# akashsengupta1997/HierarchicalProbabilistic3DHuman

Hardware: AMD Instinct MI355X
Metric: images/sec end-to-end (num_samples=100) (higher is better)
Workload: dtype f32

## Files before the change

### hierarchicalprobabilistic3dhuman_amd/csrc/api.hip

```cpp
#include <stdarg.h>

#include "hps_common.h"

namespace hps {
static thread_local char g_err[512] = "";

void set_error(const char* fmt, ...) {
    va_list ap;
    va_start(ap, fmt);
    vsnprintf(g_err, sizeof(g_err), fmt, ap);
    va_end(ap);
}
}

extern "C" int hps_version(void) { return 502; }

extern "C" int64_t hps_query_workspace(int what, int64_t d0, int64_t d1, int64_t d2) {
    if (d0 < 0 || d1 < 0 || d2 < 0) { hps::set_error("hps_query_workspace: negative dimension"); return -1; }
    const int64_t f = (int64_t)sizeof(float);
    auto up = [](int64_t x, int64_t m) { return (x + m - 1) / m * m; };
    switch (what) {
        case HPS_WS_CONV_SPLITK: return d0 <= 1 ? 0 : d0 * d1 * d2 * f;
        case HPS_WS_SMPL_MP: return up(d0, 128);
        case HPS_WS_SMPL_XT: return d1 * up(d0, 128) * f;
        case HPS_WS_SMPL_A: return d0 * d1 * 12 * f;
        case HPS_WS_SMPL_VPOSED: return d0 * up(3 * d1, 128) * f;
        case HPS_WS_HEAD_F: return d0 * d1 * 9 * f;
        case HPS_WS_HEAD_USV: return d0 * d1 * 21 * f;
        case HPS_WS_MF_LOSS: return hps::mf_loss_ws_bytes(d0);
        case HPS_WS_SMPL_LBS_BWD: return hps::lbs_backward_ws_bytes(d0, d1, d2);
        case HPS_WS_SMPL_BLEND_BWD: return hps::blend_backward_ws_bytes(d0, d1, d2);
        case HPS_WS_HEAD_LEVELS_BWD: return hps::head_levels_backward_ws_bytes(d0, d1, d2);
        case HPS_WS_HEAD_TRUNK_BWD: return hps::head_trunk_backward_ws_bytes(d0, d1, d2);
        case HPS_WS_SEG_BBOX: return d0 * 32 * 4 * (int64_t)sizeof(int32_t);
#ifdef HPS_DEV_BUILD
        case HPS_DEV_WS_HEAD_SYNC: return ((d0 + 3) / 4) * (HPS_HEAD_MAX_LEVELS + 1) * (int64_t)sizeof(int32_t);
#endif
        case HPS_WS_RENDER: return hps::render_ws_bytes(d0, d1, d2);
        case HPS_WS_SILHOUETTE: {
            const int64_t faces = d2 & 0xffffffffll, W = d2 >> 32;
            if (faces > (1 << 24) || W < 1 || W > 4096) { hps::set_error("hps_query_workspace: HPS_WS_SILHOUETTE takes d2 = faces + W * 2^32 with faces <= 2^24, W in [1, 4096]"); return -1; }
            return hps::silhouette_ws_bytes(d0, d1, faces, W);
        }
        case HPS_WS_TRAIN_METRICS: return hps::train_metrics_ws_bytes(d0);
        default: hps::set_error("hps_query_workspace: unknown item %d", what); return -1;
    }
}
extern "C" const char* hps_last_error(void) { return hps::g_err; }

extern "C" int hps_stream_create_cu_partition(int first_cu, int num_cus, hps_stream_t* stream_out) {
    if (!stream_out) return hps::bad_arg("hps_stream_create_cu_partition: null pointer");
    int dev = 0;
    hipError_t e = hipGetDevice(&dev);
    hipDeviceProp_t prop;
    if (e == hipSuccess) e = hipGetDeviceProperties(&prop, dev);
    if (e != hipSuccess) { hps::set_error("hps_stream_create_cu_partition: %s", hipGetErrorString(e)); return (int)e; }
    const int total = prop.multiProcessorCount, n_xcd = 8;
    const int per_xcd = total / n_xcd;
    if (total % n_xcd != 0 || first_cu < 0 || num_cus < 1 || first_cu + num_cus > per_xcd)
        return hps::bad_arg("hps_stream_create_cu_partition: CU range outside [0, CUs per XCD)");
    uint32_t mask[16] = {0};
    for (int c = first_cu; c < first_cu + num_cus; ++c)
        for (int x = 0; x < n_xcd; ++x) {
            const int bit = c * n_xcd + x;
            mask[bit / 32] |= 1u << (bit % 32);
        }
    hipStream_t s = nullptr;
    e = hipExtStreamCreateWithCUMask(&s, (uint32_t)((total + 31) / 32), mask);
    if (e != hipSuccess) { hps::set_error("hipExtStreamCreateWithCUMask: %s", hipGetErrorString(e)); return (int)e; }
    *stream_out = (hps_stream_t)s;
    return HPS_OK;
}

extern "C" int hps_stream_destroy(hps_stream_t stream) {
    const hipError_t e = hipStreamDestroy((hipStream_t)stream);
    if (e != hipSuccess) { hps::set_error("hipStreamDestroy: %s", hipGetErrorString(e)); return (int)e; }
    return HPS_OK;
}
```

### hierarchicalprobabilistic3dhuman_amd/csrc/conv_pad.hip

```cpp
#include <type_traits>

#include "hps_common.h"

namespace hps {

typedef float f32x16 __attribute__((ext_vector_type(16)));

constexpr int PBK = 32;

__device__ __forceinline__ unsigned fastdiv(unsigned n, unsigned d, unsigned magic) {
    unsigned q = __umulhi(n, magic);
    if (n - q * d >= d) ++q;
    return q;
}
static unsigned div_magic(unsigned d) { return d <= 1 ? 0xffffffffu : (unsigned)(0x100000000ull / d); }

__device__ __forceinline__ void lds_dma16_sv(unsigned voff, const float* sbase, unsigned lds_addr) {
    unsigned keep;
    asm volatile("s_mov_b32 %0, m0\n\ts_mov_b32 m0, %3\n\ts_nop 0\n\tglobal_load_lds_dwordx4 %1, %2\n\ts_mov_b32 m0, %0"
                 : "=&s"(keep)
                 : "v"(voff), "s"(sbase), "s"(lds_addr)
                 : "memory");
}

struct PadGeom {
    int img_pitch, row_pitch, pix_pitch;
    int cin_k;
    int kw;
    int stride, off;
    int Ho, Wo, Mtot, Kp, Cout;
    int opad;
    int relu, tiles_m, ksplit;
    unsigned magic_howo, magic_wo;
    int ablate;
};
struct DownArgs {
    const float* wn;
    const float* scale;
    const float* shift;
    float* y;
    int blocks_main;
    int tap_kh, tap_kw;
};
struct NoDown {};

#ifdef HPS_DEV_BUILD
static int g_pad_ablate = 0;
#else
constexpr int g_pad_ablate = 0;
#endif

__device__ __forceinline__ unsigned out_pixel_offset(unsigned m, const PadGeom& g) {
    const unsigned howo = (unsigned)(g.Ho * g.Wo);
    const unsigned b = fastdiv(m, howo, g.magic_howo), rem = m - b * howo;
    const unsigned ho = fastdiv(rem, (unsigned)g.Wo, g.magic_wo), wo = rem - ho * g.Wo;
    return ((b * (g.Ho + 2 * g.opad) + ho + g.opad) * (g.Wo + 2 * g.opad) + wo + g.opad) * (unsigned)g.Cout;
}

template <int BM, int BN, int WM, int WN, int ST = 2, bool DOWN = false>
__global__ __launch_bounds__(256) void conv_pad_kernel(const float* __restrict__ x, const float* __restrict__ wn,
                                                       const float* __restrict__ scale, const float* __restrict__ shift,
                                                       const float* __restrict__ residual, float* __restrict__ y,
                                                       float* __restrict__ partial, const PadGeom g,
                                                       const std::conditional_t<DOWN, DownArgs, NoDown> d) {
    constexpr int WAVES_N = BN / WN;
    constexpr int TM = WM / 32, TN = WN / 32;
    constexpr int A_LD = BM / 32, B_LD = BN / 32;
    static_assert((BM / WM) * (BN / WN) == 4, "4 waves per workgroup");
    typedef __attribute__((address_space(3))) void* lptr_t;

    extern __shared__ __attribute__((aligned(16))) float smem[];
    float* sA = smem;
    float* sB = smem + ST * BM * PBK;

    int bx = blockIdx.x;
    bool down = false;
    if constexpr (DOWN) {
        if (bx >= d.blocks_main) {
            if (blockIdx.y != 0) return;
            down = true;
            bx -= d.blocks_main;
            wn = d.wn; scale = d.scale; shift = d.shift; y = d.y; residual = nullptr;
        }
    }
    const int filter_kp = down ? g.cin_k : g.Kp;
    const int ksplit = down ? 1 : g.ksplit;
    const int relu = down ? 0 : g.relu;
    const int tile_n = bx / g.tiles_m, tile_m = bx % g.tiles_m;
    const int m0 = tile_m * BM, n0 = tile_n * BN;
    const int tid = threadIdx.x, lane = tid & 63, wave = tid >> 6;
    const int wm0 = (wave / WAVES_N) * WM, wn0 = (wave % WAVES_N) * WN;
    const int kl = lane >> 5, il = lane & 31;
    const int drow = wave * 8 + (lane >> 3);
    const int dquad = ((lane & 7) ^ ((drow >> 1) & 7)) * 4;

    unsigned a_off[A_LD], b_off[B_LD];
    {
        const unsigned howo = (unsigned)(g.Ho * g.Wo);
#pragma unroll
        for (int r = 0; r < A_LD; ++r) {
            const unsigned m = (unsigned)(m0 + drow + 32 * r);
            unsigned o = 0;
            if (m < (unsigned)g.Mtot) {
                const unsigned b = fastdiv(m, howo, g.magic_howo), rem = m - b * howo;
                const unsigned ho = fastdiv(rem, (unsigned)g.Wo, g.magic_wo), wo = rem - ho * g.Wo;
                o = b * g.img_pitch + (ho * g.stride + g.off) * g.row_pitch + (wo * g.stride + g.off) * g.pix_pitch;
            }
            a_off[r] = (o + dquad) * 4u;
        }
#pragma unroll
        for (int r = 0; r < B_LD; ++r) b_off[r] = ((unsigned)(n0 + drow + 32 * r) * filter_kp + dquad) * 4u;
    }

    f32x16 acc[TM][TN];
#pragma unroll
    for (int i = 0; i < TM; ++i)
#pragma unroll
        for (int j = 0; j < TN; ++j)
#pragma unroll
            for (int r = 0; r < 16; ++r) acc[i][j][r] = 0.0f;

    const int chunks_total = filter_kp / PBK;
    const int per_split = chunks_total / ksplit;
    const int c_begin = down ? 0 : blockIdx.y * per_split, c_end = c_begin + per_split;
    const int cpt = g.cin_k / PBK;
    int ci = c_begin % cpt, tap = c_begin / cpt;
    int kw = tap % g.kw, kh = tap / g.kw;
    if constexpr (DOWN) {
        if (down) { kh = d.tap_kh; kw = d.tap_kw; }
    }
    const float* a_src = x + (size_t)kh * g.row_pitch + (size_t)kw * g.pix_pitch + (size_t)ci * PBK;
    const float* b_src = wn + (size_t)c_begin * PBK;
    const int tap_jump = g.pix_pitch - g.cin_k + PBK;
    const int row_jump = g.row_pitch - (g.kw - 1) * g.pix_pitch - g.cin_k + PBK;

    const unsigned lds_a = (unsigned)(size_t)(lptr_t)(sA + wave * 8 * PBK);
    const unsigned lds_b = (unsigned)(size_t)(lptr_t)(sB + wave * 8 * PBK);
    auto advance = [&]() {
        b_src += PBK;
        if (++ci < cpt) a_src += PBK;
        else {
            ci = 0;
            if (++kw < g.kw) a_src += tap_jump;
            else { kw = 0; a_src += row_jump; }
        }
    };
    auto dma_chunk = [&](int buf) {
        const unsigned la = __builtin_amdgcn_readfirstlane(lds_a + buf * BM * PBK * 4);
        const unsigned lb = __builtin_amdgcn_readfirstlane(lds_b + buf * BN * PBK * 4);
#pragma unroll
        for (int r = 0; r < A_LD; ++r) lds_dma16_sv(a_off[r], a_src, la + r * 32 * PBK * 4);
#pragma unroll
        for (int r = 0; r < B_LD; ++r) lds_dma16_sv(b_off[r], b_src, lb + r * 32 * PBK * 4);
        advance();
    };
    auto dma_piece = [&](int p, const float* pa_src, const float* pb_src, unsigned la, unsigned lb) {
        if (p < A_LD) lds_dma16_sv(a_off[p < A_LD ? p : 0], pa_src, la + p * 32 * PBK * 4);
        else if (p < A_LD + B_LD) lds_dma16_sv(b_off[p >= A_LD && p < A_LD + B_LD ? p - A_LD : 0], pb_src, lb + (p - A_LD) * 32 * PBK * 4);
    };

    const int fsw = (il >> 1) & 7;
#ifdef HPS_DEV_BUILD
    if (g.ablate >= 2) {
        if (((blockIdx.x >> 8) & 1) && blockIdx.x < 512)
            for (int i = 0; i < (g.ablate - 1) * 1; ++i) __builtin_amdgcn_s_sleep(127);
    }
#endif
    dma_chunk(0);
#pragma unroll
    for (int q = 1; q < ST - 1; ++q)
        if (c_begin + q < c_end) dma_chunk(q);
    for (int c = c_begin; c < c_end; ++c) {
        const int buf = ST == 2 ? (c - c_begin) & 1 : (c - c_begin) % ST;
        {
            const int younger = min(ST - 2, c_end - 1 - c);
            if (ST >= 4 && younger >= 2) asm volatile("s_waitcnt vmcnt(%0)" ::"n"(2 * (A_LD + B_LD)) : "memory");
            else if (ST >= 3 && younger >= 1) asm volatile("s_waitcnt vmcnt(%0)" ::"n"(A_LD + B_LD) : "memory");
            else asm volatile("s_waitcnt vmcnt(0)" ::: "memory");
        }
        __syncthreads();
        static_assert(A_LD + B_LD <= (PBK / 8) * TM * TN, "one DMA piece per accumulator block of a chunk at most");
#ifdef HPS_DEV_BUILD
        const bool spread = g.ablate != 3 || ST != 2;
#else
        constexpr bool spread = true;
#endif
        const bool more = c + (ST - 1) < c_end;
        const float* na_src = a_src;
        const float* nb_src = b_src;
        const int nbuf = ST == 2 ? buf ^ 1 : (c - c_begin + ST - 1) % ST;
        const unsigned nla = __builtin_amdgcn_readfirstlane(lds_a + nbuf * BM * PBK * 4);
        const unsigned nlb = __builtin_amdgcn_readfirstlane(lds_b + nbuf * BN * PBK * 4);
        if (more) {
            if (spread) advance();
            else dma_chunk(buf ^ 1);
        }
        const float* pa = sA + (size_t)buf * BM * PBK + (wm0 + il) * PBK;
        const float* pb = sB + (size_t)buf * BN * PBK + (wn0 + il) * PBK;
        float4 a4[2][TM], b4[2][TN];
        auto load_frags = [&](int gq, int s) {
            const int slot = ((2 * gq + kl) ^ fsw) * 4;
#pragma unroll
            for (int i = 0; i < TM; ++i) a4[s][i] = *reinterpret_cast<const float4*>(pa + i * 32 * PBK + slot);
#pragma unroll
            for (int j = 0; j < TN; ++j) b4[s][j] = *reinterpret_cast<const float4*>(pb + j * 32 * PBK + slot);
        };
        load_frags(0, 0);
#pragma unroll
        for (int gq = 0; gq < PBK / 8; ++gq) {
            if (gq + 1 < PBK / 8) load_frags(gq + 1, (gq + 1) & 1);
            __builtin_amdgcn_sched_barrier(0);
#pragma unroll
            for (int i = 0; i < TM; ++i)
#pragma unroll
                for (int j = 0; j < TN; ++j) {
                    acc[i][j] = __builtin_amdgcn_mfma_f32_32x32x2f32(b4[gq & 1][j].x, a4[gq & 1][i].x, acc[i][j], 0, 0, 0);
                    acc[i][j] = __builtin_amdgcn_mfma_f32_32x32x2f32(b4[gq & 1][j].y, a4[gq & 1][i].y, acc[i][j], 0, 0, 0);
                    acc[i][j] = __builtin_amdgcn_mfma_f32_32x32x2f32(b4[gq & 1][j].z, a4[gq & 1][i].z, acc[i][j], 0, 0, 0);
                    acc[i][j] = __builtin_amdgcn_mfma_f32_32x32x2f32(b4[gq & 1][j].w, a4[gq & 1][i].w, acc[i][j], 0, 0, 0);
                    if (spread && more) {
                        __builtin_amdgcn_sched_barrier(0);
                        dma_piece((gq * TM + i) * TN + j, na_src, nb_src, nla, nlb);
                        __builtin_amdgcn_sched_barrier(0);
                    }
                }
            __builtin_amdgcn_sched_barrier(0);
        }
    }

    if (ksplit > 1) {
        float* dst = partial + (size_t)blockIdx.y * g.Mtot * g.Cout;
#pragma unroll
        for (int i = 0; i < TM; ++i) {
            const int m = m0 + wm0 + i * 32 + il;
            if (m >= g.Mtot) continue;
#pragma unroll
            for (int j = 0; j < TN; ++j)
#pragma unroll
                for (int q = 0; q < 4; ++q)
                    *reinterpret_cast<float4*>(dst + (size_t)m * g.Cout + n0 + wn0 + j * 32 + 8 * q + 4 * kl) =
                        make_float4(acc[i][j][4 * q], acc[i][j][4 * q + 1], acc[i][j][4 * q + 2], acc[i][j][4 * q + 3]);
        }
        return;
    }

    if (g.ablate == 1) {
        float t = 0.0f;
#pragma unroll
        for (int i = 0; i < TM; ++i)
#pragma unroll
            for (int j = 0; j < TN; ++j)
#pragma unroll
                for (int r = 0; r < 16; ++r) t += acc[i][j][r];
        if (t == 12345.678f) y[0] = t;
        return;
    }

    constexpr int EP = WN + 4;
    constexpr int LPP = WN / 4;
    constexpr int PPI = 64 / LPP;
    static_assert(4 * 32 * EP <= ST * (BM + BN) * PBK, "the epilogue patches fit in the K-loop buffers");
    __syncthreads();
    float* patch = smem + wave * 32 * EP;
    const int c4 = (lane % LPP) * 4;
    const int co = n0 + wn0 + c4;
    const float4 sc = *reinterpret_cast<const float4*>(scale + co), sh = *reinterpret_cast<const float4*>(shift + co);
#pragma unroll
    for (int i = 0; i < TM; ++i) {
#pragma unroll
        for (int j = 0; j < TN; ++j)
#pragma unroll
            for (int q = 0; q < 4; ++q)
                *reinterpret_cast<float4*>(patch + il * EP + j * 32 + 8 * q + 4 * kl) =
                    make_float4(acc[i][j][4 * q], acc[i][j][4 * q + 1], acc[i][j][4 * q + 2], acc[i][j][4 * q + 3]);
        constexpr int U = 32 / PPI;
        if (m0 + BM <= g.Mtot) {
            unsigned po[U];
            float4 a[U];
#pragma unroll
            for (int u = 0; u < U; ++u) {
                po[u] = out_pixel_offset((unsigned)(m0 + wm0 + i * 32 + u * PPI + lane / LPP), g) + (unsigned)co;
                a[u] = *reinterpret_cast<const float4*>(patch + (u * PPI + lane / LPP) * EP + c4);
            }
            if (residual) {
                float4 res[U];
#pragma unroll
                for (int u = 0; u < U; ++u) res[u] = *reinterpret_cast<const float4*>(residual + po[u]);
#pragma unroll
                for (int u = 0; u < U; ++u) {
                    float4 v = make_float4(a[u].x * sc.x + sh.x + res[u].x, a[u].y * sc.y + sh.y + res[u].y,
                                           a[u].z * sc.z + sh.z + res[u].z, a[u].w * sc.w + sh.w + res[u].w);
                    if (relu) { v.x = fmaxf(v.x, 0.f); v.y = fmaxf(v.y, 0.f); v.z = fmaxf(v.z, 0.f); v.w = fmaxf(v.w, 0.f); }
                    *reinterpret_cast<float4*>(y + po[u]) = v;
                }
            } else {
#pragma unroll
                for (int u = 0; u < U; ++u) {
                    float4 v = make_float4(a[u].x * sc.x + sh.x + 0.f, a[u].y * sc.y + sh.y + 0.f, a[u].z * sc.z + sh.z + 0.f,
                                           a[u].w * sc.w + sh.w + 0.f);
                    if (relu) { v.x = fmaxf(v.x, 0.f); v.y = fmaxf(v.y, 0.f); v.z = fmaxf(v.z, 0.f); v.w = fmaxf(v.w, 0.f); }
                    *reinterpret_cast<float4*>(y + po[u]) = v;
                }
            }
            continue;
        }
        unsigned po[U];
        bool live[U];
        float4 res[U];
#pragma unroll
        for (int u = 0; u < U; ++u) {
            const int m = m0 + wm0 + i * 32 + u * PPI + lane / LPP;
            live[u] = m < g.Mtot;
            po[u] = live[u] ? out_pixel_offset((unsigned)m, g) + (unsigned)co : 0u;
            res[u] = (residual && live[u]) ? *reinterpret_cast<const float4*>(residual + po[u]) : make_float4(0.f, 0.f, 0.f, 0.f);
        }
#pragma unroll
        for (int u = 0; u < U; ++u) {
            const float4 a = *reinterpret_cast<const float4*>(patch + (u * PPI + lane / LPP) * EP + c4);
            float4 v = make_float4(a.x * sc.x + sh.x + res[u].x, a.y * sc.y + sh.y + res[u].y, a.z * sc.z + sh.z + res[u].z,
                                   a.w * sc.w + sh.w + res[u].w);
            if (relu) { v.x = fmaxf(v.x, 0.f); v.y = fmaxf(v.y, 0.f); v.z = fmaxf(v.z, 0.f); v.w = fmaxf(v.w, 0.f); }
            if (live[u]) *reinterpret_cast<float4*>(y + po[u]) = v;
        }
    }
}

__global__ __launch_bounds__(256) void splitk_pad_epilogue_kernel(const float* __restrict__ partial,
                                                                  const float* __restrict__ scale,
                                                                  const float* __restrict__ shift,
                                                                  const float* __restrict__ residual,
                                                                  float* __restrict__ y, long total4, const PadGeom g) {
    const long i = (long)blockIdx.x * 256 + threadIdx.x;
    if (i >= total4) return;
    const float4* p4 = reinterpret_cast<const float4*>(partial) + i;
    float4 acc = p4[0];
    int k = 1;
    for (; k + 6 <= g.ksplit; k += 6) {
        float4 v[6];
#pragma unroll
        for (int q = 0; q < 6; ++q) v[q] = p4[(size_t)(k + q) * total4];
#pragma unroll
        for (int q = 0; q < 6; ++q) { acc.x += v[q].x; acc.y += v[q].y; acc.z += v[q].z; acc.w += v[q].w; }
    }
    for (; k < g.ksplit; ++k) {
        const float4 v = p4[(size_t)k * total4];
        acc.x += v.x; acc.y += v.y; acc.z += v.z; acc.w += v.w;
    }
    const unsigned e = (unsigned)(i * 4);
    const unsigned m = e / (unsigned)g.Cout, co = e - m * g.Cout;
    const size_t o = (size_t)out_pixel_offset(m, g) + co;
    const float4 sc = *reinterpret_cast<const float4*>(scale + co), sh = *reinterpret_cast<const float4*>(shift + co);
    float4 v = make_float4(acc.x * sc.x + sh.x, acc.y * sc.y + sh.y, acc.z * sc.z + sh.z, acc.w * sc.w + sh.w);
    if (residual) {
        const float4 r = *reinterpret_cast<const float4*>(residual + o);
        v.x += r.x; v.y += r.y; v.z += r.z; v.w += r.w;
    }
    if (g.relu) { v.x = fmaxf(v.x, 0.f); v.y = fmaxf(v.y, 0.f); v.z = fmaxf(v.z, 0.f); v.w = fmaxf(v.w, 0.f); }
    *reinterpret_cast<float4*>(y + o) = v;
}

template <int C>
__global__ __launch_bounds__(256) void nchw_to_padded_nhwc_kernel(const float* __restrict__ x, float* __restrict__ y,
                                                                  int H, int W, int P, int runs_per_row) {
    __shared__ float sp[256 * C];
    const int t = threadIdx.x;
    const int run = blockIdx.x % runs_per_row;
    const long row = blockIdx.x / runs_per_row;
    const long b = row / H;
    const int h = (int)(row - b * H);
    const int w0 = run * 256, n = min(256, W - w0);
    const long hw = (long)H * W;
    if (t < n) {
        const float* src = x + (b * C) * hw + (long)h * W + w0 + t;
#pragma unroll
        for (int c = 0; c < C; ++c) sp[t * C + c] = src[c * hw];
    }
    __syncthreads();
    float2* dst = reinterpret_cast<float2*>(y + ((b * (H + 2 * P) + h + P) * (long)(W + 2 * P) + w0 + P) * C);
    const float2* s2 = reinterpret_cast<const float2*>(sp);
    for (int i = t; i < n * C / 2; i += 256) dst[i] = s2[i];
}

__global__ __launch_bounds__(256) void nchw_to_padded_nhwc_generic_kernel(const float* __restrict__ x, float* __restrict__ y, int C,
                                                                          int CP, int H, int W, int WF, int P, long total) {
    const long i = (long)blockIdx.x * 256 + threadIdx.x;
    if (i >= total) return;
    const int w = (int)(i % W);
    long r = i / W;
    const int h = (int)(r % H); r /= H;
    const int c = (int)(r % C);
    const long b = r / C;
    y[((b * (H + 2 * P) + h + P) * (long)(WF + 2 * P) + w + P) * CP + c] = x[i];
}

__global__ __launch_bounds__(256) void maxpool_pad_kernel(const float* __restrict__ x, float* __restrict__ y, int H, int W,
                                                          int C, int Ho, int Wo, int opad, long total) {
    const long i = (long)blockIdx.x * 256 + threadIdx.x;
    if (i >= total) return;
    const int c4 = C / 4, Ho2 = (Ho + 1) / 2, Wo2 = (Wo + 1) / 2;
    const int cq = (int)(i % c4);
    long p = i / c4;
    const int wo = 2 * (int)(p % Wo2); p /= Wo2;
    const int ho = 2 * (int)(p % Ho2);
    const long b = p / Ho2;
    float4 v[5][5];
#pragma unroll
    for (int r = 0; r < 5; ++r) {
        const int hi = min(max(ho * 2 - 1 + r, 0), H - 1);
#pragma unroll
        for (int q = 0; q < 5; ++q) {
            const int wi = min(max(wo * 2 - 1 + q, 0), W - 1);
            v[r][q] = *reinterpret_cast<const float4*>(x + ((b * H + hi) * W + wi) * C + cq * 4);
        }
    }
    auto max4 = [](const float4& a, const float4& c) { return make_float4(fmaxf(a.x, c.x), fmaxf(a.y, c.y), fmaxf(a.z, c.z), fmaxf(a.w, c.w)); };
    float4 hm[5][2];
#pragma unroll
    for (int r = 0; r < 5; ++r) {
        hm[r][0] = max4(max4(v[r][0], v[r][1]), v[r][2]);
        hm[r][1] = max4(max4(v[r][2], v[r][3]), v[r][4]);
    }
#pragma unroll
    for (int a = 0; a < 2; ++a)
#pragma unroll
        for (int c = 0; c < 2; ++c) {
            if (ho + a >= Ho || wo + c >= Wo) continue;
            const float4 m = max4(max4(hm[2 * a][c], hm[2 * a + 1][c]), hm[2 * a + 2][c]);
            *reinterpret_cast<float4*>(y + ((b * (Ho + 2 * opad) + ho + a + opad) * (long)(Wo + 2 * opad) + wo + c + opad) * C + cq * 4) = m;
        }
}

__global__ __launch_bounds__(256) void avgpool_pad_kernel(const float* __restrict__ x, float* __restrict__ y, int H, int W,
                                                          int C, int P, int total) {
    const int i = blockIdx.x * 256 + threadIdx.x;
    if (i >= total) return;
    const int b = i / C, c = i % C;
    const int Wp = W + 2 * P;
    const float* s = x + ((size_t)b * (H + 2 * P) + P) * Wp * C + (size_t)P * C + c;
    float acc = 0.0f;
    for (int h = 0; h < H; ++h)
        for (int w0 = 0; w0 < W; w0 += 8) {
            float t[8];
#pragma unroll
            for (int q = 0; q < 8; ++q) t[q] = s[((size_t)h * Wp + min(w0 + q, W - 1)) * C];
#pragma unroll
            for (int q = 0; q < 8; ++q) acc += (w0 + q < W) ? t[q] : 0.0f;
        }
    y[i] = acc / (float)(H * W);
}

template <int BM, int BN, int WM, int WN, int ST = 2>
static int launch_conv_pad(const float* x, const float* wn, const float* scale, const float* shift, const float* residual,
                           float* y, float* partial, PadGeom g, hipStream_t s, const DownArgs* down = nullptr) {
    g.tiles_m = ceil_div(g.Mtot, BM);
    const int tiles_n = g.Cout / BN;
    const size_t lds = (size_t)ST * (BM + BN) * PBK * sizeof(float);
    if (down) {
        DownArgs d = *down;
        d.blocks_main = g.tiles_m * tiles_n;
        if (lds > 64 * 1024)
            if (int rc = grant_lds<&conv_pad_kernel<BM, BN, WM, WN, ST, true>>((int)lds, "hps_conv2d_bn_act_pad_down")) return rc;
        hipLaunchKernelGGL((conv_pad_kernel<BM, BN, WM, WN, ST, true>), dim3(2 * d.blocks_main, g.ksplit), dim3(256), lds, s, x, wn, scale,
                           shift, residual, y, partial, g, d);
    } else {
        if (lds > 64 * 1024)
            if (int rc = grant_lds<&conv_pad_kernel<BM, BN, WM, WN, ST>>((int)lds, "hps_conv2d_bn_act_pad")) return rc;
        hipLaunchKernelGGL((conv_pad_kernel<BM, BN, WM, WN, ST>), dim3(g.tiles_m * tiles_n, g.ksplit), dim3(256), lds, s, x, wn, scale,
                           shift, residual, y, partial, g, NoDown());
    }
    if (g.ksplit > 1) {
        const long total4 = (long)g.Mtot * g.Cout / 4;
        hipLaunchKernelGGL(splitk_pad_epilogue_kernel, dim3((unsigned)((total4 + 255) / 256)), dim3(256), 0, s, partial, scale,
                           shift, residual, y, total4, g);
    }
    return check_launch("hps_conv2d_bn_act_pad");
}

}

using namespace hps;

static int conv_pad_entry(const float* x, const float* wn, const float* scale, const float* shift,
                          const float* residual, float* y, int B, int H, int W, int ipad, int Cin, int Cout,
                          int KH, int KW, int stride, int pad, int opad, int relu, int row_mode, int variant,
                          int ksplit, float* splitk_ws, hps_stream_t stream, DownArgs* down) {
    if (!x || !wn || !scale || !shift || !y) return bad_arg("hps_conv2d_bn_act_pad: null pointer");
    if (ipad < pad || opad < 0) return bad_arg("hps_conv2d_bn_act_pad: the input halo must cover the convolution padding");
    if (Cout % 64 != 0) return bad_arg("hps_conv2d_bn_act_pad: Cout % 64 == 0 required");
    if (B <= 0) return HPS_OK;
    PadGeom g;
    const int Hp = H + 2 * ipad, Wp = W + 2 * ipad;
    g.pix_pitch = Cin;
    g.row_pitch = Wp * Cin;
    g.img_pitch = Hp * g.row_pitch;
    g.stride = stride;
    g.off = ipad - pad;
    g.Ho = (H + 2 * pad - KH) / stride + 1;
    g.Wo = (W + 2 * pad - KW) / stride + 1;
    g.Mtot = B * g.Ho * g.Wo;
    g.Cout = Cout;
    g.opad = opad;
    g.relu = relu;
    g.ksplit = ksplit < 1 ? 1 : ksplit;
    if (row_mode) {
        g.cin_k = ceil_div(KW * Cin, PBK) * PBK;
        g.kw = 1;
        if ((stride * Cin) % 4 != 0 || g.row_pitch % 4 != 0 || (g.off * Cin) % 4 != 0)
            return bad_arg("hps_conv2d_bn_act_pad: row mode needs 16-byte aligned window starts");
        if (((g.Wo - 1) * stride + g.off) * Cin + g.cin_k > g.row_pitch)
            return bad_arg("hps_conv2d_bn_act_pad: row mode window overruns the padded row");
    } else {
        if (Cin % PBK != 0) return bad_arg("hps_conv2d_bn_act_pad: Cin % 32 == 0 required (or row mode)");
        g.cin_k = Cin;
        g.kw = KW;
    }
    g.Kp = KH * g.kw * g.cin_k;
    if ((size_t)B * g.img_pitch * 4 >= 0xffffffffull || (size_t)Cout * g.Kp * 4 >= 0xffffffffull)
        return bad_arg("hps_conv2d_bn_act_pad: tensor exceeds the 32-bit lane offsets");
    if ((g.Kp / PBK) % g.ksplit != 0 || (g.ksplit > 1 && !splitk_ws)) return bad_arg("hps_conv2d_bn_act_pad: ksplit");
    g.magic_howo = div_magic((unsigned)(g.Ho * g.Wo));
    g.magic_wo = div_magic((unsigned)g.Wo);
    g.ablate = g_pad_ablate;
    hipStream_t s = (hipStream_t)stream;
    if (g.ksplit > 1 && variant != 3 && variant != 5) variant = Cout % 128 == 0 ? 1 : 2;
    if (variant == 0) {
        if (Cout % 128 == 0 && ((long)g.Mtot / 128) * (Cout / 128) >= 256) variant = 1;
        else if (Cout == 64 && g.Mtot / 256 >= 512) variant = 4;
        else variant = 3;
    }
    if (variant == 1 && Cout % 128 != 0) variant = 2;
    if (down) {
        switch (variant) {
            case 1: return launch_conv_pad<128, 128, 64, 64>(x, wn, scale, shift, residual, y, splitk_ws, g, s, down);
            case 2: return launch_conv_pad<128, 64, 64, 32>(x, wn, scale, shift, residual, y, splitk_ws, g, s, down);
            case 3: return launch_conv_pad<64, 64, 32, 32>(x, wn, scale, shift, residual, y, splitk_ws, g, s, down);
            case 5: return launch_conv_pad<64, 64, 32, 32, 4>(x, wn, scale, shift, residual, y, splitk_ws, g, s, down);
            default: set_error("hps_conv2d_bn_act_pad_down: tile variant %d carries no down-sample (issue the two convolutions separately)", variant);
                     return HPS_E_UNSUPPORTED;
        }
    }
    switch (variant) {
        case 1: return launch_conv_pad<128, 128, 64, 64>(x, wn, scale, shift, residual, y, splitk_ws, g, s);
        case 2: return launch_conv_pad<128, 64, 64, 32>(x, wn, scale, shift, residual, y, splitk_ws, g, s);
        case 3: return launch_conv_pad<64, 64, 32, 32>(x, wn, scale, shift, residual, y, splitk_ws, g, s);
        case 4: return launch_conv_pad<256, 64, 64, 64>(x, wn, scale, shift, residual, y, splitk_ws, g, s);
        case 5: return launch_conv_pad<64, 64, 32, 32, 4>(x, wn, scale, shift, residual, y, splitk_ws, g, s);
#ifdef HPS_DEV_BUILD
        case 6: return launch_conv_pad<64, 64, 32, 32, 3>(x, wn, scale, shift, residual, y, splitk_ws, g, s);
#endif
        default: return bad_arg("hps_conv2d_bn_act_pad: variant");
    }
}

extern "C" int hps_conv2d_bn_act_pad(const float* x, const float* wn, const float* scale, const float* shift,
                                     const float* residual, float* y, int B, int H, int W, int ipad, int Cin, int Cout,
                                     int KH, int KW, int stride, int pad, int opad, int relu, int row_mode, int variant,
                                     int ksplit, float* splitk_ws, hps_stream_t stream) {
    return conv_pad_entry(x, wn, scale, shift, residual, y, B, H, W, ipad, Cin, Cout, KH, KW, stride, pad, opad, relu, row_mode, variant,
                          ksplit, splitk_ws, stream, nullptr);
}

extern "C" int hps_conv2d_bn_act_pad_down(const float* x, const float* wn, const float* scale, const float* shift, float* y,
                                          const float* wn_down, const float* scale_down, const float* shift_down, float* y_down,
                                          int B, int H, int W, int ipad, int Cin, int Cout, int KH, int KW, int stride, int pad,
                                          int opad, int relu, int variant, int ksplit, float* splitk_ws, hps_stream_t stream) {
    if (!wn_down || !scale_down || !shift_down || !y_down) return bad_arg("hps_conv2d_bn_act_pad_down: null pointer");
    if (KH != KW || KH % 2 != 1 || pad != KH / 2 || stride < 1)
        return bad_arg("hps_conv2d_bn_act_pad_down: the main convolution must be k x k / s / (k / 2) (its centre tap is the 1x1 / s / 0 window)");
    DownArgs d;
    d.wn = wn_down; d.scale = scale_down; d.shift = shift_down; d.y = y_down;
    d.blocks_main = 0;
    d.tap_kh = pad; d.tap_kw = pad;
    return conv_pad_entry(x, wn, scale, shift, nullptr, y, B, H, W, ipad, Cin, Cout, KH, KW, stride, pad, opad, relu, 0, variant, ksplit,
                          splitk_ws, stream, &d);
}

#ifdef HPS_DEV_BUILD
extern "C" int hps_dev_conv_pad_ablate(int mode) {
    g_pad_ablate = mode;
    return HPS_OK;
}
#endif

extern "C" int hps_nchw_to_padded_nhwc(const float* x, float* y, int B, int C, int H, int W, int P, hps_stream_t stream) {
    if (!x || !y) return bad_arg("hps_nchw_to_padded_nhwc: null pointer");
    if (B <= 0 || H <= 0 || W <= 0) return HPS_OK;
    const int runs = ceil_div(W, 256);
    const long blocks = (long)B * H * runs;
    if (blocks > 0x7fffffffL) return bad_arg("hps_nchw_to_padded_nhwc: too many rows");
    hipStream_t s = (hipStream_t)stream;
    if (C == 18) hipLaunchKernelGGL(nchw_to_padded_nhwc_kernel<18>, dim3((unsigned)blocks), dim3(256), 0, s, x, y, H, W, P, runs);
    else if (C == 4) hipLaunchKernelGGL(nchw_to_padded_nhwc_kernel<4>, dim3((unsigned)blocks), dim3(256), 0, s, x, y, H, W, P, runs);
    else if (C == 64) hipLaunchKernelGGL(nchw_to_padded_nhwc_kernel<64>, dim3((unsigned)blocks), dim3(256), 0, s, x, y, H, W, P, runs);
    else return bad_arg("hps_nchw_to_padded_nhwc: C must be 4, 18 or 64");
    return check_launch("hps_nchw_to_padded_nhwc");
}

extern "C" int hps_nchw_to_padded_nhwc_generic(const float* x, float* y, int B, int C, int CP, int H, int W, int WF, int P,
                                               hps_stream_t stream) {
    if (!x || !y) return bad_arg("hps_nchw_to_padded_nhwc_generic: null pointer");
    if (C <= 0 || CP < C || WF < W || P < 0) return bad_arg("hps_nchw_to_padded_nhwc_generic: need CP >= C > 0, WF >= W, P >= 0");
    if (B <= 0 || H <= 0 || W <= 0) return HPS_OK;
    const long total = (long)B * C * H * W;
    if ((total + 255) / 256 > 0x7fffffffL) return bad_arg("hps_nchw_to_padded_nhwc_generic: tensor too large");
    hipLaunchKernelGGL(nchw_to_padded_nhwc_generic_kernel, dim3((unsigned)((total + 255) / 256)), dim3(256), 0, (hipStream_t)stream, x, y,
                       C, CP, H, W, WF, P, total);
    return check_launch("hps_nchw_to_padded_nhwc_generic");
}

extern "C" int hps_maxpool3x3s2_pad(const float* x, float* y, int B, int H, int W, int C, int opad, hps_stream_t stream) {
    if (!x || !y) return bad_arg("hps_maxpool3x3s2_pad: null pointer");
    if (C % 4 != 0) return bad_arg("hps_maxpool3x3s2_pad: C % 4 == 0 required");
    const int Ho = (H + 2 - 3) / 2 + 1, Wo = (W + 2 - 3) / 2 + 1;
    const long total = (long)B * ((Ho + 1) / 2) * ((Wo + 1) / 2) * (C / 4);
    if (total <= 0) return HPS_OK;
    hipLaunchKernelGGL(maxpool_pad_kernel, dim3((unsigned)((total + 255) / 256)), dim3(256), 0, (hipStream_t)stream, x, y, H, W,
                       C, Ho, Wo, opad, total);
    return check_launch("hps_maxpool3x3s2_pad");
}

extern "C" int hps_global_avgpool_pad(const float* x, float* y, int B, int H, int W, int C, int P, hps_stream_t stream) {
    if (!x || !y) return bad_arg("hps_global_avgpool_pad: null pointer");
    const int total = B * C;
    if (total <= 0) return HPS_OK;
    hipLaunchKernelGGL(avgpool_pad_kernel, dim3((total + 255) / 256), dim3(256), 0, (hipStream_t)stream, x, y, H, W, C, P,
                       total);
    return check_launch("hps_global_avgpool_pad");
}
```

### hierarchicalprobabilistic3dhuman_amd/csrc/hps_common.h

```cpp
#pragma once
#include <hip/hip_runtime.h>
#include <stdint.h>
#include <stdio.h>

#include <atomic>

#include "hps.h"
#ifdef HPS_DEV_BUILD
#include "hps_dev.h"
#endif

namespace hps {

void set_error(const char* fmt, ...);

int64_t mf_loss_ws_bytes(int64_t rows);
int64_t lbs_backward_ws_bytes(int64_t M, int64_t V, int64_t J);
int64_t blend_backward_ws_bytes(int64_t M, int64_t kp, int64_t np);
int64_t head_levels_backward_ws_bytes(int64_t B, int64_t total_in, int64_t NJ);
int64_t head_trunk_backward_ws_bytes(int64_t B, int64_t wide, int64_t nt);
int64_t render_ws_bytes(int64_t B, int64_t Nd, int64_t F);
int64_t silhouette_ws_bytes(int64_t M, int64_t Nd, int64_t F, int64_t W);
int64_t train_metrics_ws_bytes(int64_t B);

inline int check_launch(const char* what) {
    hipError_t e = hipGetLastError();
    if (e != hipSuccess) {
        set_error("%s: %s", what, hipGetErrorString(e));
        return (int)e;
    }
    return HPS_OK;
}

inline int bad_arg(const char* what) {
    set_error("bad argument: %s", what);
    return HPS_E_BADARG;
}

__host__ __device__ inline int ceil_div(int a, int b) { return (a + b - 1) / b; }

template <auto Kernel>
inline int grant_lds(int bytes, const char* what) {
    static std::atomic<uint64_t> granted{0};
    int dev = 0;
    hipError_t e = hipGetDevice(&dev);
    if (e == hipSuccess && dev < 64 && ((granted.load(std::memory_order_acquire) >> dev) & 1ull)) return HPS_OK;
    if (e == hipSuccess)
        e = hipFuncSetAttribute(reinterpret_cast<const void*>(Kernel), hipFuncAttributeMaxDynamicSharedMemorySize, bytes);
    if (e != hipSuccess) {
        set_error("%s: granting %d bytes of dynamic LDS failed: %s", what, bytes, hipGetErrorString(e));
        return (int)e;
    }
    if (dev < 64) granted.fetch_or(1ull << dev, std::memory_order_release);
    return HPS_OK;
}

struct __attribute__((packed, aligned(4))) f3 {
    float x, y, z;
};

__device__ __forceinline__ float det3(const float* m) {
    return m[0] * (m[4] * m[8] - m[5] * m[7]) - m[1] * (m[3] * m[8] - m[5] * m[6]) +
           m[2] * (m[3] * m[7] - m[4] * m[6]);
}

__device__ __forceinline__ void mat3_mul(const float* a, const float* b, float* c) {
#pragma unroll
    for (int i = 0; i < 3; ++i)
#pragma unroll
        for (int j = 0; j < 3; ++j)
            c[i * 3 + j] = a[i * 3 + 0] * b[0 * 3 + j] + a[i * 3 + 1] * b[1 * 3 + j] + a[i * 3 + 2] * b[2 * 3 + j];
}

__device__ __forceinline__ void mat3_mul_bt(const float* a, const float* b, float* c) {
#pragma unroll
    for (int i = 0; i < 3; ++i)
#pragma unroll
        for (int j = 0; j < 3; ++j)
            c[i * 3 + j] = a[i * 3 + 0] * b[j * 3 + 0] + a[i * 3 + 1] * b[j * 3 + 1] + a[i * 3 + 2] * b[j * 3 + 2];
}

__device__ __forceinline__ void quat_to_rotmat_dev(float qw, float qx, float qy, float qz, float* r) {
    float n = sqrtf(qw * qw + qx * qx + qy * qy + qz * qz);
    float w = qw / n, x = qx / n, y = qy / n, z = qz / n;
    float w2 = w * w, x2 = x * x, y2 = y * y, z2 = z * z;
    float wx = w * x, wy = w * y, wz = w * z, xy = x * y, xz = x * z, yz = y * z;
    r[0] = w2 + x2 - y2 - z2; r[1] = 2 * xy - 2 * wz;     r[2] = 2 * wy + 2 * xz;
    r[3] = 2 * wz + 2 * xy;   r[4] = w2 - x2 + y2 - z2;   r[5] = 2 * yz - 2 * wx;
    r[6] = 2 * xz - 2 * wy;   r[7] = 2 * wx + 2 * yz;     r[8] = w2 - x2 - y2 + z2;
}

__device__ __forceinline__ void rodrigues_dev(float rx, float ry, float rz, float* r) {
    float ex = rx + 1e-8f, ey = ry + 1e-8f, ez = rz + 1e-8f;
    float angle = sqrtf(ex * ex + ey * ey + ez * ez);
    float dx = rx / angle, dy = ry / angle, dz = rz / angle;
    float s = sinf(angle), c = 1.0f - cosf(angle);
    float k[9] = {0.f, -dz, dy, dz, 0.f, -dx, -dy, dx, 0.f};
    float k2[9];
    mat3_mul(k, k, k2);
#pragma unroll
    for (int i = 0; i < 9; ++i) r[i] = ((i % 4 == 0) ? 1.0f : 0.0f) + s * k[i] + c * k2[i];
}


template <int K>
__device__ __forceinline__ f3 skin_vertex(const float* Am, const int (&idx)[K], const float (&w)[K], const f3 pv, float tx,
                                          float ty, float tz) {
    typedef float v2f __attribute__((ext_vector_type(2)));
    v2f P[6];
#pragma unroll
    for (int e = 0; e < 6; ++e) P[e] = (v2f){0.0f, 0.0f};
#pragma unroll
    for (int k = 0; k < K; ++k) {
        const float4* t4 = reinterpret_cast<const float4*>(Am + idx[k]);
        const float4 r0 = t4[0], r1 = t4[1], r2 = t4[2];
        const v2f wk = (v2f){w[k], w[k]};
        P[0] = __builtin_elementwise_fma(wk, (v2f){r0.x, r0.y}, P[0]);
        P[1] = __builtin_elementwise_fma(wk, (v2f){r0.z, r0.w}, P[1]);
        P[2] = __builtin_elementwise_fma(wk, (v2f){r1.x, r1.y}, P[2]);
        P[3] = __builtin_elementwise_fma(wk, (v2f){r1.z, r1.w}, P[3]);
        P[4] = __builtin_elementwise_fma(wk, (v2f){r2.x, r2.y}, P[4]);
        P[5] = __builtin_elementwise_fma(wk, (v2f){r2.z, r2.w}, P[5]);
    }
    const float T[12] = {P[0].x, P[0].y, P[1].x, P[1].y, P[2].x, P[2].y, P[3].x, P[3].y, P[4].x, P[4].y, P[5].x, P[5].y};
    f3 o;
    o.x = __builtin_fmaf(T[2], pv.z, __builtin_fmaf(T[1], pv.y, T[0] * pv.x)) + T[3] + tx;
    o.y = __builtin_fmaf(T[6], pv.z, __builtin_fmaf(T[5], pv.y, T[4] * pv.x)) + T[7] + ty;
    o.z = __builtin_fmaf(T[10], pv.z, __builtin_fmaf(T[9], pv.y, T[8] * pv.x)) + T[11] + tz;
    return o;
}

__device__ __forceinline__ float div3_rn(float v) {
    const float inv = 0.3333333432674407958984375f;
    const float q = v * inv;
    const float r = __builtin_fmaf(-3.0f, q, v);
    return r == 0.0f ? q : __builtin_fmaf(r, inv, q);
}

__device__ __forceinline__ void lds_dma16(unsigned voff, const float* sbase, unsigned lds_addr) {
    unsigned keep;
    lds_addr = __builtin_amdgcn_readfirstlane(lds_addr);
    asm volatile("s_mov_b32 %0, m0\n\ts_mov_b32 m0, %3\n\ts_nop 0\n\tglobal_load_lds_dwordx4 %1, %2\n\ts_mov_b32 m0, %0"
                 : "=&s"(keep)
                 : "v"(voff), "s"(sbase), "s"(lds_addr)
                 : "memory");
}

}
```

Before: 22510.

## Add in-launch split-K reduction, templated second-pass epilogue, small-map pooling path

Adds an optional FIN variant of the padded conv kernel in which the last split-K workgroup for a tile, picked through an atomic ticket counter, reduces the partial slices and applies BN, residual and ReLU, removing the separate epilogue launch. That path is only compiled in dev builds and only taken under an ablation flag, so by default the second-pass epilogue still runs. The epilogue is now templated on common ksplit values so its loads fully unroll, and it uses 64-thread blocks for small outputs. Global average pooling gains a fully unrolled 8x8 path for small spatial maps. The fused path costs extra counter workspace and depends on fence ordering between workgroups.

```diff
diff --git a/hierarchicalprobabilistic3dhuman_amd/csrc/api.hip b/hierarchicalprobabilistic3dhuman_amd/csrc/api.hip
--- a/hierarchicalprobabilistic3dhuman_amd/csrc/api.hip
+++ b/hierarchicalprobabilistic3dhuman_amd/csrc/api.hip
@@ -20,7 +20,7 @@
     const int64_t f = (int64_t)sizeof(float);
     auto up = [](int64_t x, int64_t m) { return (x + m - 1) / m * m; };
     switch (what) {
-        case HPS_WS_CONV_SPLITK: return d0 <= 1 ? 0 : d0 * d1 * d2 * f;
+        case HPS_WS_CONV_SPLITK: return hps::conv_splitk_ws_bytes(d0, d1, d2);
         case HPS_WS_SMPL_MP: return up(d0, 128);
         case HPS_WS_SMPL_XT: return d1 * up(d0, 128) * f;
         case HPS_WS_SMPL_A: return d0 * d1 * 12 * f;
diff --git a/hierarchicalprobabilistic3dhuman_amd/csrc/conv_pad.hip b/hierarchicalprobabilistic3dhuman_amd/csrc/conv_pad.hip
--- a/hierarchicalprobabilistic3dhuman_amd/csrc/conv_pad.hip
+++ b/hierarchicalprobabilistic3dhuman_amd/csrc/conv_pad.hip
@@ -57,7 +57,14 @@
     return ((b * (g.Ho + 2 * g.opad) + ho + g.opad) * (g.Wo + 2 * g.opad) + wo + g.opad) * (unsigned)g.Cout;
 }
 
-template <int BM, int BN, int WM, int WN, int ST = 2, bool DOWN = false>
+__device__ __forceinline__ float4 splitk_bn_act4(const float4 acc, const float4 sc, const float4 sh, bool has_res, const float4 r, int relu) {
+    float4 v = make_float4(acc.x * sc.x + sh.x, acc.y * sc.y + sh.y, acc.z * sc.z + sh.z, acc.w * sc.w + sh.w);
+    if (has_res) { v.x += r.x; v.y += r.y; v.z += r.z; v.w += r.w; }
+    if (relu) { v.x = fmaxf(v.x, 0.f); v.y = fmaxf(v.y, 0.f); v.z = fmaxf(v.z, 0.f); v.w = fmaxf(v.w, 0.f); }
+    return v;
+}
+
+template <int BM, int BN, int WM, int WN, int ST = 2, bool DOWN = false, bool FIN = false>
 __global__ __launch_bounds__(256) void conv_pad_kernel(const float* __restrict__ x, const float* __restrict__ wn,
                                                        const float* __restrict__ scale, const float* __restrict__ shift,
                                                        const float* __restrict__ residual, float* __restrict__ y,
@@ -241,6 +248,74 @@
                     *reinterpret_cast<float4*>(dst + (size_t)m * g.Cout + n0 + wn0 + j * 32 + 8 * q + 4 * kl) =
                         make_float4(acc[i][j][4 * q], acc[i][j][4 * q + 1], acc[i][j][4 * q + 2], acc[i][j][4 * q + 3]);
         }
+        if constexpr (FIN) {
+            int* cnt = reinterpret_cast<int*>(partial + (size_t)ksplit * g.Mtot * g.Cout) + bx;
+            asm volatile("s_waitcnt vmcnt(0)" ::: "memory");
+            __syncthreads();
+            int* is_last = reinterpret_cast<int*>(smem);
+            if (tid == 0) {
+                __builtin_amdgcn_fence(__ATOMIC_RELEASE, "agent");
+                asm volatile("s_waitcnt vmcnt(0)" ::: "memory");
+                const int ticket = __hip_atomic_fetch_add(cnt, 1, __ATOMIC_RELAXED, __HIP_MEMORY_SCOPE_AGENT);
+                const int last = ticket == ksplit - 1;
+                if (last) {
+                    __hip_atomic_store(cnt, 0, __ATOMIC_RELAXED, __HIP_MEMORY_SCOPE_AGENT);
+                    __builtin_amdgcn_fence(__ATOMIC_ACQUIRE, "agent");
+                    asm volatile("s_waitcnt vmcnt(0)" ::: "memory");
+                }
+                *is_last = last;
+            }
+            __syncthreads();
+            if (!*is_last) return;
+            constexpr int Q = BN / 4;
+            constexpr int NG = BM * BN / 4 / 256;
+            constexpr int GB = NG < 4 ? NG : 4;
+            constexpr int SB = 6;
+            const size_t slice4 = (size_t)g.Mtot * g.Cout / 4;
+#pragma unroll
+            for (int g0 = 0; g0 < NG; g0 += GB) {
+                const float4* p[GB];
+                unsigned mm[GB], cc[GB];
+                float4 a[GB];
+#pragma unroll
+                for (int u = 0; u < GB; ++u) {
+                    const int e = (g0 + u) * 256 + tid;
+                    mm[u] = (unsigned)(m0 + e / Q);
+                    cc[u] = (unsigned)(n0 + (e % Q) * 4);
+                    const unsigned src_m = mm[u] < (unsigned)g.Mtot ? mm[u] : (unsigned)m0;
+                    p[u] = reinterpret_cast<const float4*>(partial + (size_t)src_m * g.Cout + cc[u]);
+                }
+#pragma unroll
+                for (int u = 0; u < GB; ++u) a[u] = p[u][0];
+                int k = 1;
+                for (; k + SB <= ksplit; k += SB) {
+                    float4 v[GB][SB];
+#pragma unroll
+                    for (int q = 0; q < SB; ++q)
+#pragma unroll
+                        for (int u = 0; u < GB; ++u) v[u][q] = p[u][(size_t)(k + q) * slice4];
+#pragma unroll
+                    for (int q = 0; q < SB; ++q)
+#pragma unroll
+                        for (int u = 0; u < GB; ++u) { a[u].x += v[u][q].x; a[u].y += v[u][q].y; a[u].z += v[u][q].z; a[u].w += v[u][q].w; }
+                }
+                for (; k < ksplit; ++k) {
+                    float4 v[GB];
+#pragma unroll
+                    for (int u = 0; u < GB; ++u) v[u] = p[u][(size_t)k * slice4];
+#pragma unroll
+                    for (int u = 0; u < GB; ++u) { a[u].x += v[u].x; a[u].y += v[u].y; a[u].z += v[u].z; a[u].w += v[u].w; }
+                }
+#pragma unroll
+                for (int u = 0; u < GB; ++u)
+                    if (mm[u] < (unsigned)g.Mtot) {
+                        const size_t o = (size_t)out_pixel_offset(mm[u], g) + cc[u];
+                        const float4 sc = *reinterpret_cast<const float4*>(scale + cc[u]), sh = *reinterpret_cast<const float4*>(shift + cc[u]);
+                        const float4 r = residual ? *reinterpret_cast<const float4*>(residual + o) : make_float4(0.f, 0.f, 0.f, 0.f);
+                        *reinterpret_cast<float4*>(y + o) = splitk_bn_act4(a[u], sc, sh, residual != nullptr, r, relu);
+                    }
+            }
+        }
         return;
     }
 
@@ -325,38 +400,48 @@
     }
 }
 
+template <int KS>
 __global__ __launch_bounds__(256) void splitk_pad_epilogue_kernel(const float* __restrict__ partial,
                                                                   const float* __restrict__ scale,
                                                                   const float* __restrict__ shift,
                                                                   const float* __restrict__ residual,
                                                                   float* __restrict__ y, long total4, const PadGeom g) {
-    const long i = (long)blockIdx.x * 256 + threadIdx.x;
+    const long i = (long)blockIdx.x * blockDim.x + threadIdx.x;
     if (i >= total4) return;
     const float4* p4 = reinterpret_cast<const float4*>(partial) + i;
-    float4 acc = p4[0];
-    int k = 1;
-    for (; k + 6 <= g.ksplit; k += 6) {
-        float4 v[6];
-#pragma unroll
-        for (int q = 0; q < 6; ++q) v[q] = p4[(size_t)(k + q) * total4];
-#pragma unroll
-        for (int q = 0; q < 6; ++q) { acc.x += v[q].x; acc.y += v[q].y; acc.z += v[q].z; acc.w += v[q].w; }
-    }
-    for (; k < g.ksplit; ++k) {
-        const float4 v = p4[(size_t)k * total4];
-        acc.x += v.x; acc.y += v.y; acc.z += v.z; acc.w += v.w;
-    }
     const unsigned e = (unsigned)(i * 4);
     const unsigned m = e / (unsigned)g.Cout, co = e - m * g.Cout;
     const size_t o = (size_t)out_pixel_offset(m, g) + co;
-    const float4 sc = *reinterpret_cast<const float4*>(scale + co), sh = *reinterpret_cast<const float4*>(shift + co);
-    float4 v = make_float4(acc.x * sc.x + sh.x, acc.y * sc.y + sh.y, acc.z * sc.z + sh.z, acc.w * sc.w + sh.w);
-    if (residual) {
-        const float4 r = *reinterpret_cast<const float4*>(residual + o);
-        v.x += r.x; v.y += r.y; v.z += r.z; v.w += r.w;
-    }
-    if (g.relu) { v.x = fmaxf(v.x, 0.f); v.y = fmaxf(v.y, 0.f); v.z = fmaxf(v.z, 0.f); v.w = fmaxf(v.w, 0.f); }
-    *reinterpret_cast<float4*>(y + o) = v;
+    float4 acc, sc, sh, r = make_float4(0.f, 0.f, 0.f, 0.f);
+    if constexpr (KS > 0) {
+        float4 v[KS];
+#pragma unroll
+        for (int k = 0; k < KS; ++k) v[k] = p4[(size_t)k * total4];
+        sc = *reinterpret_cast<const float4*>(scale + co);
+        sh = *reinterpret_cast<const float4*>(shift + co);
+        if (residual) r = *reinterpret_cast<const float4*>(residual + o);
+        acc = v[0];
+#pragma unroll
+        for (int k = 1; k < KS; ++k) { acc.x += v[k].x; acc.y += v[k].y; acc.z += v[k].z; acc.w += v[k].w; }
+    } else {
+        acc = p4[0];
+        int k = 1;
+        for (; k + 6 <= g.ksplit; k += 6) {
+            float4 v[6];
+#pragma unroll
+            for (int q = 0; q < 6; ++q) v[q] = p4[(size_t)(k + q) * total4];
+#pragma unroll
+            for (int q = 0; q < 6; ++q) { acc.x += v[q].x; acc.y += v[q].y; acc.z += v[q].z; acc.w += v[q].w; }
+        }
+        for (; k < g.ksplit; ++k) {
+            const float4 v = p4[(size_t)k * total4];
+            acc.x += v.x; acc.y += v.y; acc.z += v.z; acc.w += v.w;
+        }
+        sc = *reinterpret_cast<const float4*>(scale + co);
+        sh = *reinterpret_cast<const float4*>(shift + co);
+        if (residual) r = *reinterpret_cast<const float4*>(residual + o);
+    }
+    *reinterpret_cast<float4*>(y + o) = splitk_bn_act4(acc, sc, sh, residual != nullptr, r, g.relu);
 }
 
 template <int C>
@@ -438,6 +523,19 @@
     const int Wp = W + 2 * P;
     const float* s = x + ((size_t)b * (H + 2 * P) + P) * Wp * C + (size_t)P * C + c;
     float acc = 0.0f;
+    if (H <= 8 && W <= 8 && total <= 8192) {
+        float t[8][8];
+#pragma unroll
+        for (int r = 0; r < 8; ++r)
+#pragma unroll
+            for (int q = 0; q < 8; ++q) t[r][q] = s[((size_t)min(r, H - 1) * Wp + min(q, W - 1)) * C];
+#pragma unroll
+        for (int r = 0; r < 8; ++r)
+#pragma unroll
+            for (int q = 0; q < 8; ++q) acc += (r < H && q < W) ? t[r][q] : 0.0f;
+        y[i] = acc / (float)(H * W);
+        return;
+    }
     for (int h = 0; h < H; ++h)
         for (int w0 = 0; w0 < W; w0 += 8) {
             float t[8];
@@ -447,6 +545,38 @@
             for (int q = 0; q < 8; ++q) acc += (w0 + q < W) ? t[q] : 0.0f;
         }
     y[i] = acc / (float)(H * W);
+}
+
+enum { PAD_FORCE_IN_LAUNCH = 101, PAD_FORCE_SECOND_PASS = 102, PAD_FORCE_IN_LAUNCH_ZEROED = 103 };
+#ifdef HPS_DEV_BUILD
+constexpr bool FIN_BUILT = true;
+__global__ __launch_bounds__(256) void zero_ints_kernel(int* __restrict__ p, int n) {
+    const int i = blockIdx.x * 256 + threadIdx.x;
+    if (i < n) p[i] = 0;
+}
+#else
+constexpr bool FIN_BUILT = false;
+#endif
+static bool splitk_in_launch(int64_t ksplit) {
+    return FIN_BUILT && ksplit > 1 && (g_pad_ablate == PAD_FORCE_IN_LAUNCH || g_pad_ablate == PAD_FORCE_IN_LAUNCH_ZEROED);
+}
+
+int64_t conv_splitk_ws_bytes(int64_t ksplit, int64_t M, int64_t Cout) {
+    if (ksplit <= 1) return 0;
+    const int64_t slices = ksplit * M * Cout * (int64_t)sizeof(float);
+    const int64_t counters = ((M + 63) / 64 * ((Cout + 63) / 64) + 3) / 4 * 4;
+    return splitk_in_launch(ksplit) ? slices + counters * (int64_t)sizeof(int) : slices;
+}
+
+template <int BM, int BN, int WM, int WN, int ST, bool DOWN, bool FIN, class D>
+static int launch_conv_pad_kernel(dim3 grid, const float* x, const float* wn, const float* scale, const float* shift,
+                                  const float* residual, float* y, float* partial, const PadGeom& g, hipStream_t s, const D& d) {
+    const size_t lds = (size_t)ST * (BM + BN) * PBK * sizeof(float);
+    if (lds > 64 * 1024)
+        if (int rc = grant_lds<&conv_pad_kernel<BM, BN, WM, WN, ST, DOWN, FIN>>((int)lds, DOWN ? "hps_conv2d_bn_act_pad_down" : "hps_conv2d_bn_act_pad"))
+            return rc;
+    hipLaunchKernelGGL((conv_pad_kernel<BM, BN, WM, WN, ST, DOWN, FIN>), grid, dim3(256), lds, s, x, wn, scale, shift, residual, y, partial, g, d);
+    return HPS_OK;
 }
 
 template <int BM, int BN, int WM, int WN, int ST = 2>
@@ -454,24 +584,49 @@
                            float* y, float* partial, PadGeom g, hipStream_t s, const DownArgs* down = nullptr) {
     g.tiles_m = ceil_div(g.Mtot, BM);
     const int tiles_n = g.Cout / BN;
-    const size_t lds = (size_t)ST * (BM + BN) * PBK * sizeof(float);
+    constexpr bool can_finish = FIN_BUILT && BM <= 128 && ST != 3;
+    const bool fin = can_finish && splitk_in_launch(g.ksplit);
+#ifdef HPS_DEV_BUILD
+    if (fin && g_pad_ablate != PAD_FORCE_IN_LAUNCH_ZEROED) {
+        int* cnt = reinterpret_cast<int*>(partial + (size_t)g.ksplit * g.Mtot * g.Cout);
+        const int ints = g.tiles_m * tiles_n;
+        hipLaunchKernelGGL(zero_ints_kernel, dim3(ceil_div(ints, 256)), dim3(256), 0, s, cnt, ints);
+    }
+#endif
+    int rc = HPS_OK;
     if (down) {
         DownArgs d = *down;
         d.blocks_main = g.tiles_m * tiles_n;
-        if (lds > 64 * 1024)
-            if (int rc = grant_lds<&conv_pad_kernel<BM, BN, WM, WN, ST, true>>((int)lds, "hps_conv2d_bn_act_pad_down")) return rc;
-        hipLaunchKernelGGL((conv_pad_kernel<BM, BN, WM, WN, ST, true>), dim3(2 * d.blocks_main, g.ksplit), dim3(256), lds, s, x, wn, scale,
-                           shift, residual, y, partial, g, d);
+        const dim3 grid(2 * d.blocks_main, g.ksplit);
+        if constexpr (can_finish) {
+            if (fin) rc = launch_conv_pad_kernel<BM, BN, WM, WN, ST, true, true>(grid, x, wn, scale, shift, residual, y, partial, g, s, d);
+        }
+        if (!fin) rc = launch_conv_pad_kernel<BM, BN, WM, WN, ST, true, false>(grid, x, wn, scale, shift, residual, y, partial, g, s, d);
     } else {
-        if (lds > 64 * 1024)
-            if (int rc = grant_lds<&conv_pad_kernel<BM, BN, WM, WN, ST>>((int)lds, "hps_conv2d_bn_act_pad")) return rc;
-        hipLaunchKernelGGL((conv_pad_kernel<BM, BN, WM, WN, ST>), dim3(g.tiles_m * tiles_n, g.ksplit), dim3(256), lds, s, x, wn, scale,
-                           shift, residual, y, partial, g, NoDown());
-    }
-    if (g.ksplit > 1) {
+        const dim3 grid(g.tiles_m * tiles_n, g.ksplit);
+        if constexpr (can_finish) {
+            if (fin) rc = launch_conv_pad_kernel<BM, BN, WM, WN, ST, false, true>(grid, x, wn, scale, shift, residual, y, partial, g, s, NoDown());
+        }
+        if (!fin) rc = launch_conv_pad_kernel<BM, BN, WM, WN, ST, false, false>(grid, x, wn, scale, shift, residual, y, partial, g, s, NoDown());
+    }
+    if (rc != HPS_OK) return rc;
+    if (g.ksplit > 1 && !fin) {
         const long total4 = (long)g.Mtot * g.Cout / 4;
-        hipLaunchKernelGGL(splitk_pad_epilogue_kernel, dim3((unsigned)((total4 + 255) / 256)), dim3(256), 0, s, partial, scale,
-                           shift, residual, y, total4, g);
+        const unsigned bs2 = total4 <= 65536 ? 64u : 256u;
+        const dim3 grid2((unsigned)((total4 + bs2 - 1) / bs2));
+        switch (g.ksplit) {
+#define HPS_SECOND_PASS(KS) hipLaunchKernelGGL(splitk_pad_epilogue_kernel<KS>, grid2, dim3(bs2), 0, s, partial, scale, shift, residual, y, total4, g)
+            case 2: HPS_SECOND_PASS(2); break;
+            case 3: HPS_SECOND_PASS(3); break;
+            case 4: HPS_SECOND_PASS(4); break;
+            case 6: HPS_SECOND_PASS(6); break;
+            case 8: HPS_SECOND_PASS(8); break;
+            case 9: HPS_SECOND_PASS(9); break;
+            case 12: HPS_SECOND_PASS(12); break;
+            case 18: HPS_SECOND_PASS(18); break;
+            default: HPS_SECOND_PASS(0); break;
+#undef HPS_SECOND_PASS
+        }
     }
     return check_launch("hps_conv2d_bn_act_pad");
 }
@@ -520,7 +675,7 @@
     if ((g.Kp / PBK) % g.ksplit != 0 || (g.ksplit > 1 && !splitk_ws)) return bad_arg("hps_conv2d_bn_act_pad: ksplit");
     g.magic_howo = div_magic((unsigned)(g.Ho * g.Wo));
     g.magic_wo = div_magic((unsigned)g.Wo);
-    g.ablate = g_pad_ablate;
+    g.ablate = g_pad_ablate >= PAD_FORCE_IN_LAUNCH ? 0 : g_pad_ablate;
     hipStream_t s = (hipStream_t)stream;
     if (g.ksplit > 1 && variant != 3 && variant != 5) variant = Cout % 128 == 0 ? 1 : 2;
     if (variant == 0) {
diff --git a/hierarchicalprobabilistic3dhuman_amd/csrc/hps_common.h b/hierarchicalprobabilistic3dhuman_amd/csrc/hps_common.h
--- a/hierarchicalprobabilistic3dhuman_amd/csrc/hps_common.h
+++ b/hierarchicalprobabilistic3dhuman_amd/csrc/hps_common.h
@@ -14,6 +14,7 @@
 
 void set_error(const char* fmt, ...);
 
+int64_t conv_splitk_ws_bytes(int64_t ksplit, int64_t M, int64_t Cout);
 int64_t mf_loss_ws_bytes(int64_t rows);
 int64_t lbs_backward_ws_bytes(int64_t M, int64_t V, int64_t J);
 int64_t blend_backward_ws_bytes(int64_t M, int64_t kp, int64_t np);
```

New measurement: 22510 (median of 2 runs). No clear change (+0.0%).
